# yyNoBug/VAE_segmentation

Hardware: AMD Instinct MI355X
Metric: 3D train-step volumes/sec at 96^3 batch=2 (joint VAE+seg) (higher is better)
Workload: dtype bf16; 1 GPU; configs[1]: 96^3 joint VAE+seg training step (joint_train), batch=2/GPU, bf16 activations + fp32 accumulate, SGD momentum 0.9, VAE frozen, HIP-graph replay; global_batch=2, parallelism=dp1, activation_recomputation=False, tail_in_graph=True, nranks=1, grad_exchange=none (1 rank)

## Files before the change

include/vaeseg.h:

```cpp
#ifndef VAESEG_H
#define VAESEG_H
#include <stddef.h>
#include <stdint.h>

#ifdef __cplusplus
extern "C" {
#endif

#define VS_VERSION 500

enum { VS_F32 = 0, VS_BF16 = 1, VS_F16 = 2, VS_F32X3 = 3  };
#ifndef VS_STAT_SLOTS
#define VS_STAT_SLOTS 4
#endif
enum { VS_OK = 0, VS_EINVAL = -1, VS_ESHAPE = -2, VS_EDTYPE = -3, VS_EWORKSPACE = -4, VS_EALIGN = -5 };

enum {
    VS_CONV_K3 = 0,
    VS_CONV_K2S2 = 1,
    VS_CONV_T2S2 = 2,
    VS_WGRAD_SLABS = 16,
    VS_CONV_UP = 3
};

// ... 85 lines not shown
    long long wgrad_f32_tiles;
    long long wgrad_group_wgs;
    long long wgrad_big_min_voxels;
} vs_config;
int vs_config_bytes(void);
int vs_config_from_env(vs_config* c);
int vs_get_config(vs_config* out);
int vs_set_config(const vs_config* cfg);
int vs_conv_k3_bwd_data_applied_supported(int n, int d, int h, int w, int c_in, int m_out, int dtype);
int vs_conv_k3_bwd_data_applied(const void* x, const void* w_packed, void* y, const void* mask_x, const double* mask_stats, double* sums,
                                unsigned int* sync, unsigned int* fault, int n, int d, int h, int w, int c_in, int m_out, int dtype, float eps, void* stream);
int vs_conv_s2_bwd_data_applied_supported(int n, int d, int h, int w, int c_in, int m_out, int scatter, int dtype);
int vs_conv_s2_bwd_data_applied(const void* x, const void* w_packed, void* y, const void* mask_x, const double* mask_stats, double* sums, const void* add,
                                unsigned int* sync, unsigned int* fault, int n, int d, int h, int w, int c_in, int m_out, int scatter, int dtype, float eps,
                                void* stream);
typedef struct vs_chain_layer {
    const void* x;
    const double* x_stats;
    const void* w_packed;
    void* y;
    double* y_stats;
    const void* mask_x;
    const double* mask_stats;
    double* sums;
    int c_in, m_out;
    int apply;
    int reserved_;
} vs_chain_layer;
int vs_conv_k3_chain_supported(int n, int d, int h, int w, int c_max, int dtype);
long long vs_conv_k3_chain_sync_bytes(int n);
// ... 35 lines not shown
int vs_bias_grad_acc(const void* g, float* db, long long rows, int c_ch, int c_real, int dtype, int accumulate, void* stream);

int vs_instnorm_stats(const void* x, double* stats, int n, long long voxels, int c, int dtype, void* stream);
int vs_instnorm_relu_fwd(const void* x, const double* x_stats, const void* x2, const double* x2_stats,
                         void* out, int n, long long voxels, int c, int dtype, float eps, void* stream);
int vs_instnorm_relu_bwd_reduce(const void* g, const void* x, const double* x_stats, double* sums,
                                int n, long long voxels, int c, int dtype, float eps, void* stream);
int vs_instnorm_relu_bwd_apply(const void* g, const void* x, const double* x_stats, const double* sums,
                               void* gx, int n, long long voxels, int c, int dtype, float eps, void* stream);
int vs_instnorm_relu_bwd_apply_add(const void* g, const void* x, const double* x_stats, const double* sums, const void* add,
                                   void* gx, int n, long long voxels, int c, int dtype, float eps, void* stream);
int vs_zero_fill(void* p, long long bytes, void* stream);
int vs_instnorm_relu_bwd_pair(const void* g, const void* x1, const double* x1_stats, double* sums1, void* gx1,
                              const void* x2, const double* x2_stats, double* sums2, void* gx2, int n, long long voxels,
                              int c, int dtype, float eps, void* stream);

enum { VS_NORM_INSTANCE = 0, VS_NORM_BATCH = 1, VS_NORM_BATCH_EVAL = 2, VS_NORM_NONE = 3 };
enum { VS_ACT_RELU = 0, VS_ACT_SOFTPLUS = 1 };
int vs_norm_tables(const double* stats, int n, int c, int c_real, double count, int mode, float eps, float momentum,
                   float* running_mean, float* running_var, long long* num_batches_tracked, float* mean, float* rstd, void* stream);
int vs_norm_act_fwd(const void* x, const float* mean, const float* rstd, const float* gamma, const float* beta, void* y, int n,
                    long long voxels, int c, int c_real, int act, int dtype, void* stream);
int vs_norm_act_bwd_reduce(const void* g, const void* x, const float* mean, const float* rstd, const float* gamma, const float* beta,
                           double* sums, int n, long long voxels, int c, int c_real, int act, int dtype, void* stream);
int vs_norm_act_bwd_finish(const double* sums, int n, int c, int c_real, double count, int mode, const float* rstd, const float* gamma,
                           float* coef, float* dgamma, float* dbeta, void* stream);
int vs_norm_act_bwd_apply(const void* g, const void* x, const float* mean, const float* rstd, const float* gamma, const float* beta,
                          const float* coef, void* dx, int n, long long voxels, int c, int c_real, int act, int dtype, void* stream);

int vs_gsnorm_fwd(const void* x, void* y, long long rows, int c, int num_group, int dtype, void* stream);
// ... 197 lines not shown
```

vae_segmentation_amd/csrc/conv_api.hip:

```cpp
#include <stdlib.h>
#include "igemm_dispatch.h"

int g1_dispatch_k3_f32(const G1Params& p, int ck, int mt, int epi, int tiles, int row_tiles, hipStream_t s);
int g1_dispatch_k3_bf16(const G1Params& p, int ck, int mt, int epi, int tiles, int row_tiles, hipStream_t s);
int g1_dispatch_k3_f16(const G1Params& p, int ck, int mt, int epi, int tiles, int row_tiles, hipStream_t s);
int g1_dispatch_k3_x3(const G1Params& p, int ck, int mt, int epi, int tiles, int row_tiles, hipStream_t s);
int g1_k3_fa_supported(const G1Params& p, int ck, int mt, int lazy_in);
int g1_k3_ea_supported(const G1Params& p, int ck, int mt, long long wgs);
int k3x_fa_supported(const G1Params& p, int ck, int mt);
int k3x_ea_supported(const G1Params& p, int ck, int mt, long long wgs);
int k3tw_slab_count(int n, int d, int h, int w);
int k2s2_scatter8_launch(const G1Params& p, int dtype, hipStream_t stream);

extern "C" int vs_conv_k3_f32_limbs(int d, int h, int w, int c_in) {
    const int on = vs_cfg().f32_limbs;
    if (!on) return 0;
    const int small = vs_cfg().k3_small;
    if (small && c_in % 32 == 0 && c_in <= 1024 && (long long)(d + 2) * (h + 2) * (w + 2) <= 512) return 0;
    return 1;
}

struct ConvTiles { int ck, mt, row_tiles; bool limbs; };

static ConvTiles k3_tiles(G1Params& p, int dtype, int ck, int mt, int rows16, long long tiles) {
// ... 30 lines not shown
static inline bool wide_layer(int c_in, int m_out) { return c_in > 256 || m_out > 256; }

static int shape_status(int n, int d, int h, int w_, int c_in, int dtype, bool misaligned = false) {
    if (n <= 0 || d <= 0 || h <= 0 || w_ <= 0) return VS_ESHAPE;
    if (!(c_in == 8 || c_in == 16 || (c_in % 32 == 0 && c_in > 0 && c_in <= VS_MAX_CHANNELS))) return VS_ESHAPE;
    if (!vs_dtype_ok(dtype)) return VS_EDTYPE;
    if (misaligned) return VS_EALIGN;
    return (double)n * d * h * w_ * c_in >= 2147483648.0 ? VS_ESHAPE : VS_OK;
}

static int check_common(const void* x, const void* w, int n, int d, int h, int w_, int c_in, int dtype) {
    if (!x || !w) return VS_EINVAL;
    return shape_status(n, d, h, w_, c_in, dtype, ((uintptr_t)x & 15) || ((uintptr_t)w & 15));
}

enum { X_STATS = 1, BIAS = 2, SUMS = 4, FA = 8, WGRAD = 16, EA = 32 };
struct ConvAsk { int n, d, h, w, c_in, m_out, kind, dtype, parts; };

struct ConvPlan {
    ConvAsk ask;
    G1Params g;
    ConvTiles t;
    long long tiles;
    int status;
    bool fa_ok, ea_ok, wg_ok;
    bool stream8;
};

static void g1_ea_plan(ConvPlan& pl, long long wgs) {
    pl.ea_ok = pl.t.mt == 16 && wgs <= 256;
    if (pl.ask.parts & EA) pl.g.ea_items = pl.g.tiles_per_sample * pl.t.row_tiles;
}

static ConvPlan plan_begin(const ConvAsk& a, int rows) {
    ConvPlan pl{};
    pl.ask = a;
    pl.status = shape_status(a.n, a.d, a.h, a.w, a.c_in, a.dtype);
    if (!pl.status && (a.m_out <= 0 || a.m_out % 8)) pl.status = VS_EINVAL;
    if (!pl.status && a.m_out > VS_MAX_CHANNELS) pl.status = VS_ESHAPE;
    if (pl.status) return pl;
    G1Params& p = pl.g;
    p.N = a.n; p.D = a.d; p.H = a.h; p.W = a.w;
    p.C = a.c_in; p.M = a.m_out;
    p.rb_total = (rows + 15) / 16;
    pl.t.ck = a.c_in < 32 ? a.c_in : 32;
    p.nch = a.c_in / pl.t.ck;
    p.inv_count_in = 1.0 / ((double)a.d * a.h * a.w);
    return pl;
}

static ConvPlan plan_gather(const ConvAsk& a) {
    ConvPlan pl = plan_begin(a, a.m_out);
    const bool k3 = a.kind == VS_CONV_K3, sums = a.parts & SUMS, fa = a.parts & FA, ea = a.parts & EA;
    if (!pl.status && !k3 && a.kind != VS_CONV_K2S2) pl.status = VS_EINVAL;
    if (!pl.status && wide_layer(a.c_in, a.m_out) && (a.parts & (EA | FA | WGRAD))) pl.status = VS_ESHAPE;
    if (!pl.status && !k3 && ((a.d | a.h | a.w) & 1)) pl.status = VS_ESHAPE;
    if (pl.status) return pl;
    G1Params& p = pl.g;
    const int ck = pl.t.ck;
    if (k3) {
        p.Do = a.d; p.Ho = a.h; p.Wo = a.w;
        p.tyn = (a.h + 3) / 4; p.txn = (a.w + 15) / 16;
        p.tiles_per_sample = ((a.d + 3) / 4) * p.tyn * p.txn;
    } else {
        p.Do = a.d / 2; p.Ho = a.h / 2; p.Wo = a.w / 2;
        p.tiles_per_sample = vs_ceil_div((long long)p.Do * p.Ho * p.Wo, 256);
        if (ck == 32 && p.nch >= 2 && (long long)p.tiles_per_sample * a.n * p.rb_total <= 64) {
            p.tiles_per_sample = vs_ceil_div((long long)p.Do * p.Ho * p.Wo, 64);
            p.tyn = 64;
        }
// ... 5 lines not shown
    if (k3 && fa && ck == 32 && mt == 16 && rows16 % 32 == 0) mt = 32;
    pl.t = k3 ? k3_tiles(p, a.dtype, ck, mt, rows16, pl.tiles) : ConvTiles{ck, mt, rows16 / mt, false};
    const long long wgs = pl.tiles * pl.t.row_tiles;
    if (!k3) {
        g1_ea_plan(pl, wgs);
    } else if (a.dtype != VS_F32) {
        pl.fa_ok = g1_k3_fa_supported(p, pl.t.ck, pl.t.mt, sums) != 0;
        pl.ea_ok = g1_k3_ea_supported(p, pl.t.ck, pl.t.mt, wgs) != 0;
        pl.wg_ok = vs_cfg().fuse_wgrad && a.c_in == 8 && a.m_out == 8 && a.n * 8 <= 192 && (double)a.n * a.d * a.h * a.w * 16 < 2147483648.0 &&
                   vs_k3_toeplitz(8, 8, 27, a.dtype);
    } else if (pl.t.limbs) {
        pl.fa_ok = k3x_fa_supported(p, pl.t.ck, pl.t.mt) != 0;
        pl.ea_ok = k3x_ea_supported(p, pl.t.ck, pl.t.mt, wgs) != 0;
    }
    pl.ea_ok = pl.ea_ok && sums && !fa && vs_cfg().epilogue_apply;
    if ((fa && !pl.fa_ok) || (ea && !pl.ea_ok) || ((a.parts & WGRAD) && !pl.wg_ok)) pl.status = VS_ESHAPE;
    return pl;
}

static ConvPlan plan_scatter(const ConvAsk& a) {
    ConvPlan pl = plan_begin(a, 8 * a.m_out);
    const bool sums = a.parts & SUMS, ea = a.parts & EA;
    if (!pl.status && wide_layer(a.c_in, a.m_out) && ea) pl.status = VS_ESHAPE;
    if (pl.status) return pl;
    G1Params& p = pl.g;
    p.Do = a.d; p.Ho = a.h; p.Wo = a.w;
    p.inv_count_out = 1.0 / (8.0 * a.d * a.h * a.w);
    p.tiles_per_sample = vs_ceil_div((long long)a.d * a.h * a.w, 256);
    pl.tiles = (long long)p.tiles_per_sample * a.n;
    pl.stream8 = !ea && vs_cfg().k2s2_stream && sums && a.c_in == 8 && a.m_out == 8 && a.dtype != VS_F32 && !(a.parts & (BIAS | X_STATS));
    const int rows16 = p.rb_total * 16;
// ... 140 lines not shown
    return plan_s2_applied(n, d, h, w, c_in, m_out, scatter, dtype).status == VS_OK;
}

extern "C" int vs_conv_s2_bwd_data_applied(const void* x, const void* w_packed, void* y, const void* mask_x, const double* mask_stats, double* sums, const void* add,
                                           unsigned int* sync, unsigned int* fault, int n, int d, int h, int w, int c_in, int m_out, int scatter, int dtype, float eps,
                                           void* stream) {
    if (!mask_x || !mask_stats || !sums || !sync || !fault) return VS_EINVAL;
    if (((uintptr_t)sync & 127) || ((uintptr_t)fault & 3) || (add && ((uintptr_t)add & 15))) return VS_EALIGN;
    const ConvPlan pl = plan_s2_applied(n, d, h, w, c_in, m_out, scatter, dtype);
    if (pl.status) return VS_ESHAPE;
    G1Params p = bwd_params(pl, x, w_packed, y, mask_x, mask_stats, sums, eps);
    p.ea_sync = sync; p.ea_fault = fault; p.ea_add = add;
    return launch_conv(pl, p, stream);
}

extern "C" int vs_conv_k3_softmax2_fwd(const void* x, const double* x_stats, const void* w_packed, const float* bias,
                                       float* prob, int n, int d, int h, int w, int c_in, int dtype, float eps,
                                       void* stream) {
    return vs_conv_k3_softmax2_dropout_fwd(x, x_stats, w_packed, bias, prob, n, d, h, w, c_in, dtype, eps, 0.f, 0ull, stream);
}

extern "C" int vs_conv_k3_softmax2_dropout_fwd(const void* x, const double* x_stats, const void* w_packed, const float* bias,
                                               float* prob, int n, int d, int h, int w, int c_in, int dtype, float eps,
                                               float drop_p, unsigned long long drop_seed, void* stream) {
    return vs_conv_k3_softmax2_cl_fwd(x, x_stats, w_packed, bias, prob, nullptr, n, d, h, w, c_in, dtype, eps, drop_p, drop_seed, stream);
}

extern "C" int vs_conv_k3_softmax2_cl_fwd(const void* x, const double* x_stats, const void* w_packed, const float* bias, float* prob, void* prob_cl,
                                          int n, int d, int h, int w, int c_in, int dtype, float eps, float drop_p, unsigned long long drop_seed, void* stream) {
    if (drop_p < 0.f || drop_p >= 1.f) return VS_EINVAL;
// ... 12 lines not shown
```

vae_segmentation_amd/csrc/igemm.h:

```cpp
#pragma once
#include <type_traits>
#include "common.h"
#include "handoff.h"

enum { G1_K3 = 0, G1_K2S2 = 1, G1_PW = 2 };
enum { EPI_RAW = 0, EPI_SOFTMAX2 = 1, EPI_SCATTER = 2 };

struct G1Params {
    const void* x;
    const double* x_stats;
    const void* wp;
    const float* bias;
    void* y;
    double* y_stats;
    float* prob;
    const void* mask_x;
    const double* mask_stats;
    double* sums;
    double inv_count_out;
    float drop_p;
    unsigned long long drop_seed;
    int N, D, H, W;
    int Do, Ho, Wo;
    int C;
    int M;
    int rb_total;
    int nch;
    int tiles_per_sample;
    int tyn, txn;
    float eps;
    double inv_count_in;
    unsigned int fd_m[3], fd_s[3];
    const void* fa_x;
    const double* fa_sums;
    void* fa_dx;
    const void* up_taps;
    const float* up_btab;
    int up_co;
    float* wg_ws;
    const float* sm_prob;
    const float* sm_gprob;
    const void* sm_gcl;
    double* wg_bias;
    unsigned int* ea_sync;
    unsigned int* ea_fault;
    int ea_items;
    const void* ea_add;
};

#define G1_LDS_MEAN 0
#define G1_LDS_RSTD 2048
#define G1_LDS_RED 4096
#define G1_LDS_BYTES 6144
#define G1_TILE_VOX 648

template <typename T, int CK>
__device__ __forceinline__ u32x4 act_transform(u32x4 raw, const float* s_mean, const float* s_rstd, int c0) {
    constexpr int EPL = ET<T>::EPL;
    float v[EPL];
    frag_unpack(raw, v, (T*)nullptr);
#pragma unroll
    for (int j = 0; j < EPL; ++j) {
        float t = (v[j] - s_mean[c0 + j]) * s_rstd[c0 + j];
        v[j] = t > 0.f ? t : 0.f;
    }
    return frag_pack(v, (T*)nullptr);
}

template <typename T, int CK, int KIND, int MT, int EPI, bool LIMB = false, bool EA = false>
__global__ __launch_bounds__(256) void g1_kernel(const G1Params p) {
    using E = ET<T>;
    constexpr int EPL = E::EPL, KG = E::KG;
    static_assert(!LIMB || sizeof(T) == 4, "limb arithmetic: fp32 storage");
    static_assert(KIND == G1_K2S2 || KIND == G1_PW, "the 3x3x3 kernels live in igemm_k3b.h / igemm_k3.h");
    static_assert(EPI == EPI_RAW || EPI == EPI_SCATTER, "softmax epilogue: 3x3x3 kernels only");
    constexpr int NTAPS = KIND == G1_K2S2 ? 8 : 1;
    constexpr int NKG = (NTAPS * CK + KG - 1) / KG;
    constexpr int RB = MT / 16;
    constexpr int CKB = CK * (int)sizeof(T);
    constexpr int TPK = KG > CK ? KG / CK : 1;
    constexpr int KPT = KG > CK ? 1 : CK / KG;
    extern __shared__ __attribute__((aligned(16))) char smem[];
    float* s_mean = (float*)(smem + G1_LDS_MEAN);
    float* s_rstd = (float*)(smem + G1_LDS_RSTD);
    float* s_red = (float*)(smem + G1_LDS_RED);

    const int tid = threadIdx.x;
    const int lane = tid & 63;
    const int wave = tid >> 6;
    const int col = lane & 15;
    const int g = lane >> 4;
    const int n = blockIdx.x / p.tiles_per_sample;
    const int tile = blockIdx.x - n * p.tiles_per_sample;
    const int rb0 = blockIdx.y * RB;
    const bool has_stats = p.x_stats != nullptr;
    const T* __restrict__ xin = (const T*)p.x;

    if (has_stats) {
        for (int c = tid; c < p.C; c += 256) {
            float m, r;
            stats_to_mean_rstd(p.x_stats, (size_t)n * p.C + c, (size_t)p.N * p.C, p.inv_count_in, p.eps, m, r);
            s_mean[c] = m;
            s_rstd[c] = r;
        }
    }
    if (p.sums != nullptr) {
        for (int c = tid; c < p.M; c += 256) {
            float m, r;
            stats_to_mean_rstd(p.mask_stats, (size_t)n * p.M + c, (size_t)p.N * p.M, p.inv_count_out, p.eps, m, r);
            s_mean[c] = m;
            s_rstd[c] = r;
        }
    }
    const bool splitw = KIND == G1_K2S2 && CK == 32 && p.tyn == 64;
    const int cwave = splitw ? 0 : wave;
    const int ctile = splitw ? 64 : 256;
    long long gofs[4];
    bool cvalid[4];
    int oz[4], oy[4], ox[4];
    {
        const int vcol = p.Do * p.Ho * p.Wo;
#pragma unroll
        for (int cg = 0; cg < 4; ++cg) {
            int v = tile * ctile + cwave * 64 + cg * 16 + col;
            cvalid[cg] = v < vcol;
            if (!cvalid[cg]) v = 0;
// ... 247 lines not shown

    auto out_elem = [&](int rb, int cg, int& m_out, bool& valid) -> size_t {
        const int row = (rb0 + rb) * 16 + 4 * g;
        int m = row, tap = 0;
        if constexpr (EPI == EPI_SCATTER) { tap = row / p.M; m = row - tap * p.M; }
        const bool rvalid = EPI == EPI_SCATTER ? (tap < 8) : (row < p.M);
        m_out = m;
        valid = rvalid && cvalid[cg];
        if constexpr (EPI == EPI_SCATTER) {
            const int dz = (tap >> 2) & 1, dy = (tap >> 1) & 1, dx = tap & 1;
            return ((((size_t)n * (2 * p.D) + 2 * oz[cg] + dz) * (2 * p.H) + 2 * oy[cg] + dy) * (2 * p.W) + 2 * ox[cg] + dx) * p.M + m;
        } else {
            return ((((size_t)n * p.Do + oz[cg]) * p.Ho + oy[cg]) * p.Wo + ox[cg]) * p.M + m;
        }
    };
    constexpr int MKW = sizeof(T) == 4 ? 4 : 2;
    unsigned int mkv[RB][4][MKW];
    constexpr bool ea = EA;
    static_assert(!EA || MT == 16, "epilogue apply: 16-row workgroups");
    unsigned int adv[EA ? RB : 1][4][MKW];
    if (p.sums != nullptr) {
#pragma unroll
        for (int rb = 0; rb < RB; ++rb)
#pragma unroll
            for (int cg = 0; cg < 4; ++cg) {
                int m; bool ok;
                const size_t e = out_elem(rb, cg, m, ok);
#pragma unroll
                for (int i = 0; i < MKW; ++i) { mkv[rb][cg][i] = 0u; if constexpr (EA) adv[rb][cg][i] = 0u; }
                if (ok) {
// ... 132 lines not shown
                float xv[4], av[4], o[4];
                widen4<T>(mkv[rb][cg], xv);
                widen4<T>(adv[rb][cg], av);
#pragma unroll
                for (int r = 0; r < 4; ++r) {
                    const float gv = E::rnd(acc[rb][cg][r] + bvq[rb][r]);
                    o[r] = vs_in_bwd_apply1(gv, xv[r], tb[r][0], tb[r][1], tb[r][2], tb[r][3]);
                    if (p.ea_add != nullptr) o[r] = E::rnd(o[r]) + av[r];
                }
                store4<T>(yout + e, o);
            }
        }
    }
}

template <typename T, int CK, int KIND, int MT, int EPI, bool LIMB = false, bool EA = false>
static int g1_launch(const G1Params& p, int tiles_total, int row_tiles, hipStream_t stream) {
    constexpr size_t lds = G1_LDS_BYTES + (KIND == G1_K2S2 && CK == 32 ? (size_t)3 * (MT / 16) * 4 * 64 * 16 : 0);
    auto kern = g1_kernel<T, CK, KIND, MT, EPI, LIMB, EA>;
    hipLaunchKernelGGL(kern, dim3(tiles_total, row_tiles), dim3(256), lds, stream, p);
    VS_CHECK_LAUNCH();
    return VS_OK;
}
```

vae_segmentation_amd/csrc/igemm_dispatch.h:

```cpp
#pragma once
#include "igemm.h"

int g1_dispatch_k2s2(const G1Params& p, int dtype, int ck, int mt, int tiles, int row_tiles, hipStream_t s);
int g1_dispatch_pw(const G1Params& p, int dtype, int ck, int mt, int tiles, int row_tiles, hipStream_t s);

#define G1_CASE(T, CKV, KIND, MTV, EPI) \
    if (ck == CKV && mt == MTV) return g1_launch<T, CKV, KIND, MTV, EPI>(p, tiles, row_tiles, s);

#define G1_ALL_MT(T, CKV, KIND, EPI) \
    G1_CASE(T, CKV, KIND, 16, EPI) G1_CASE(T, CKV, KIND, 32, EPI) G1_CASE(T, CKV, KIND, 64, EPI)

#define G1_ALL(T, KIND, EPI) G1_ALL_MT(T, 8, KIND, EPI) G1_ALL_MT(T, 16, KIND, EPI) G1_ALL_MT(T, 32, KIND, EPI)
#define G1L_CASE(CKV, KIND, MTV, EPI) \
    if (ck == CKV && mt == MTV) return g1_launch<float, CKV, KIND, MTV, EPI, true>(p, tiles, row_tiles, s);
#define G1L_ALL_MT(CKV, KIND, EPI) G1L_CASE(CKV, KIND, 16, EPI) G1L_CASE(CKV, KIND, 32, EPI) G1L_CASE(CKV, KIND, 64, EPI)
#define G1L_ALL(KIND, EPI) G1L_ALL_MT(8, KIND, EPI) G1L_ALL_MT(16, KIND, EPI) G1L_ALL_MT(32, KIND, EPI)
#define G1E_ALL(T, KIND, EPI, LIMBV) \
    if (p.ea_sync != nullptr) { \
        if (mt == 16 && ck == 8) return g1_launch<T, 8, KIND, 16, EPI, LIMBV, true>(p, tiles, row_tiles, s); \
        if (mt == 16 && ck == 16) return g1_launch<T, 16, KIND, 16, EPI, LIMBV, true>(p, tiles, row_tiles, s); \
        if (mt == 16 && ck == 32) return g1_launch<T, 32, KIND, 16, EPI, LIMBV, true>(p, tiles, row_tiles, s); \
        return VS_ESHAPE; \
    }
static inline bool g1_f32_limbs() {
    const int on = vs_cfg().f32_limbs;
    const int g1 = vs_cfg().g1_limbs;
    return on != 0 && g1 != 0;
}
```

vae_segmentation_amd/csrc/igemm_g1_f16.hip:

```cpp
#include "igemm_dispatch.h"
int g1_dispatch_k2s2_f16(const G1Params& p, int ck, int mt, int tiles, int row_tiles, hipStream_t s) {
    G1E_ALL(vs_half, G1_K2S2, EPI_RAW, false)
    G1_ALL(vs_half, G1_K2S2, EPI_RAW)
    return VS_ESHAPE;
}
int g1_dispatch_pw_f16(const G1Params& p, int ck, int mt, int tiles, int row_tiles, hipStream_t s) {
    G1E_ALL(vs_half, G1_PW, EPI_SCATTER, false)
    G1_ALL(vs_half, G1_PW, EPI_SCATTER)
    return VS_ESHAPE;
}
```

vae_segmentation_amd/csrc/igemm_k2s2.hip:

```cpp
#include <stdlib.h>
#include "igemm_dispatch.h"
int g1_dispatch_k2s2_f16(const G1Params& p, int ck, int mt, int tiles, int row_tiles, hipStream_t s);
int g1_dispatch_k2s2(const G1Params& p, int dtype, int ck, int mt, int tiles, int row_tiles, hipStream_t s) {
    if (dtype == VS_F32) { if (g1_f32_limbs()) { G1E_ALL(float, G1_K2S2, EPI_RAW, true) G1L_ALL(G1_K2S2, EPI_RAW) } else { G1E_ALL(float, G1_K2S2, EPI_RAW, false) G1_ALL(float, G1_K2S2, EPI_RAW) } }
    else if (dtype == VS_BF16) { G1E_ALL(unsigned short, G1_K2S2, EPI_RAW, false) G1_ALL(unsigned short, G1_K2S2, EPI_RAW) }
    else if (dtype == VS_F16) return g1_dispatch_k2s2_f16(p, ck, mt, tiles, row_tiles, s);
    return VS_ESHAPE;
}
```

vae_segmentation_amd/csrc/norm.hip:

```cpp
#include "common.h"

#define NB_MAX_C 512

template <typename T>
struct RowIter {
    int fx, fy, frags, rows_per_it;
    __device__ RowIter(int c) {
        frags = c / ET<T>::EPL;
        fx = threadIdx.x % frags;
        fy = threadIdx.x / frags;
        rows_per_it = 256 / frags;
    }
    __device__ bool active() const { return fy < rows_per_it; }
};

__device__ __forceinline__ void load_mean_rstd(const double* stats, int n, int c, double inv_count, float eps,
                                               float* s_mean, float* s_rstd) {
    const size_t pairs = (size_t)gridDim.y * c;
    for (int i = threadIdx.x; i < c; i += blockDim.x) {
        float m = 0.f, r = 1.f;
        if (stats) stats_to_mean_rstd(stats, (size_t)n * c + i, pairs, inv_count, eps, m, r);
        s_mean[i] = m;
        s_rstd[i] = r;
    }
// ... 340 lines not shown
extern "C" int vs_instnorm_relu_bwd_pair(const void* g, const void* x1, const double* x1_stats, double* sums1, void* gx1,
                                         const void* x2, const double* x2_stats, double* sums2, void* gx2, int n, long long voxels,
                                         int c, int dtype, float eps, void* stream) {
    int rc = check_cl(x1, n, voxels, c, dtype);
    if (rc) return rc;
    if (!g || !x2 || !x1_stats || !x2_stats || !sums1 || !sums2 || !gx1 || !gx2) return VS_EINVAL;
    InBwdPair a;
    a.x[0] = x1; a.x[1] = x2; a.xs[0] = x1_stats; a.xs[1] = x2_stats; a.sums[0] = sums1; a.sums[1] = sums2; a.gx[0] = gx1; a.gx[1] = gx2;
    const double inv = 1.0 / (double)voxels;
    dim3 grid(row_blocks(voxels, c, dtype), n, 2);
    dispatch_t(dtype, [&](auto* tag) {
        using T = TAG_T(tag);
        hipLaunchKernelGGL(in_relu_bwd_reduce2_kernel<T>, grid, dim3(256), red_lds(dtype, 2), (hipStream_t)stream, (const T*)g, a, voxels, c, inv, eps);
    });
    VS_CHECK_LAUNCH();
    const int rpi = 256 / (c / (dtype == VS_F32 ? 4 : 8));
    long long gb = (voxels + (long long)rpi * 4 - 1) / ((long long)rpi * 4);
    const long long gcap = 2048 / (2 * n) > 0 ? 2048 / (2 * n) : 1;
    if (gb > gcap) gb = gcap;
    dim3 grid2((unsigned)gb, n, 2);
    dispatch_t(dtype, [&](auto* tag) {
        using T = TAG_T(tag);
        hipLaunchKernelGGL(in_relu_bwd_apply2_kernel<T>, grid2, dim3(256), 0, (hipStream_t)stream, (const T*)g, a, voxels, c, inv, eps);
    });
    VS_CHECK_LAUNCH();
    return VS_OK;
}

extern "C" int vs_bias_grad(const void* g, float* db, long long rows, int c_ch, int c_real, int dtype, void* stream) {
    return vs_bias_grad_acc(g, db, rows, c_ch, c_real, dtype, 0, stream);
// ... 286 lines not shown
```

vae_segmentation_amd/modules.py:

```python
import torch
import torch.nn as nn

from . import ops

_DEFAULT_DTYPE = torch.float32


def set_default_kernel_dtype(dtype):
    global _DEFAULT_DTYPE
    if dtype not in ops.KERNEL_DTYPES:
        raise TypeError("kernel dtype must be torch.float32, torch.bfloat16 or torch.float16")
    _DEFAULT_DTYPE = dtype


def set_kernel_dtype(module, dtype):
    if dtype not in ops.KERNEL_DTYPES:
        raise TypeError("kernel dtype must be torch.float32, torch.bfloat16 or torch.float16")
    for m in module.modules():
        if hasattr(m, "kernel_dtype"):
            m.kernel_dtype = dtype
    return module


class Act:
# ... 106 lines not shown
        a = _conv_norm_act(self.conv, 0, a)
        return _as_tensor(a, self.out_ch) if wrapped else a


class Up(nn.Module):

    def __init__(self, in_ch, out_ch, norm_type=2, kernal_size=(2, 2, 2), stride=(2, 2, 2), soft=False):
        super().__init__()
        if tuple(kernal_size) != (2, 2, 2) or tuple(stride) != (2, 2, 2):
            raise NotImplementedError("native transposed conv is written for kernel 2, stride 2")
        self.conv = nn.Sequential(nn.ConvTranspose3d(in_ch, in_ch, kernal_size, stride=stride, padding=0),
                                  DoubleConv(in_ch, out_ch, norm_type, soft=False))
        self.out_ch = out_ch
        self.kernel_dtype = _DEFAULT_DTYPE

    def forward(self, x):
        a, wrapped = _as_act(x, self.kernel_dtype)
        t, dc = self.conv[0], self.conv[1]
        if dc.lazy_head() and ops.up_composed_ok(a.raw, t, dc.conv[0]):
            y, ys = ops.UpConvK3.apply(a.raw, a.stats, t.weight, t.bias, dc.conv[0].weight, dc.conv[0].bias)
            a = dc(Act(y, ys), _start=3)
        else:
            a = dc(Act(ops.ConvT2S2.apply(a.raw, a.stats, t.weight, t.bias), None))
        return _as_tensor(a, self.out_ch) if wrapped else a


class Down(nn.Module):

    def __init__(self, in_ch, out_ch, norm_type=2, kernal_size=(2, 2, 2), stride=(2, 2, 2), soft=False):
        super().__init__()
        if tuple(kernal_size) != (2, 2, 2) or tuple(stride) != (2, 2, 2):
            raise NotImplementedError("native strided conv is written for kernel 2, stride 2")
        self.conv = nn.Sequential(nn.Conv3d(in_ch, in_ch, kernal_size, stride=stride, padding=0),
# ... 16 lines not shown
    enabled = bool(enabled)
    if enabled == _RECOMPUTE[0]:
        return
    _RECOMPUTE[0] = enabled
    if enabled:
        _RECOMPUTE_SAVED_GROUPING[0] = bool(ops._GROUP["enabled"])
        ops.set_wgrad_grouping(False)
    else:
        ops.set_wgrad_grouping(_RECOMPUTE_SAVED_GROUPING[0])


def _has_training_batchnorm(blk):
    return any(isinstance(m, nn.BatchNorm3d) and m.training for m in blk.modules())


def _run_block(blk, a):
    if not (_RECOMPUTE[0] and torch.is_grad_enabled() and a.raw.requires_grad):
        return blk(a)
    if _has_training_batchnorm(blk):
        return blk(a)
    from torch.utils.checkpoint import checkpoint

    def run(raw, stats):
        out = blk(Act(raw, stats))
        return out.raw, out.stats

    marks = getattr(a.raw, "_vs_defer_apply", False)

    def run_marked(raw, stats):
        if marks:
            raw._vs_defer_apply = True
        return run(raw, stats)

    raw, stats = checkpoint(run_marked, a.raw, a.stats, use_reentrant=False, preserve_rng_state=False)
    return Act(raw, stats)


def _check_n_class(n_class):
    if not 1 <= int(n_class) <= 8:
        raise NotImplementedError("native softmax / label kernels hold n_class in one 8-channel fragment: 1..8, got %r" % (n_class,))


def _dropout(a, p):
    if not p:
        return a
    x = ops.Materialize.apply(a.raw, a.stats, None, None) if a.stats is not None else a.raw
    return Act(ops.Dropout.apply(x, float(p), ops.next_dropout_seed()), None)


# ... 91 lines not shown

    def forward(self, data_dict, in_key, out_key, dropout=0.0):
        x = data_dict[in_key]
        ops._require_cuda(x)
        if any(s % 16 for s in x.shape[2:]):
            raise ValueError("Segmentation needs spatial sizes that are multiples of 16, got %s" % (tuple(x.shape[2:]),))
        ops.stats_arena_begin(x.device)
        a = Act(ops.PackPlanar.apply(x, self.kernel_dtype), None)
        x1 = self.in_block(a)
        x2 = _run_block(self.down1, x1)
        x3 = _run_block(self.down2, x2)
        x4 = _run_block(self.down3, x3)
        x5 = _run_block(self.down4, x4)
        u = _dropout(_run_block(self.up2, x5), dropout)
        u = _run_block(self.up3, u)
        u = _dropout(Act(ops.Materialize.apply(u.raw, u.stats, x3.raw, x3.stats, True), None), dropout)
        u = _run_block(self.up4, u)
        u = _dropout(Act(ops.Materialize.apply(u.raw, u.stats, x2.raw, x2.stats, True), None), dropout)
        u = _dropout(_run_block(self.up5, u), dropout)
        if u.stats is not None:
            ops.mark_defer_apply(u.raw, self.up5.conv[1].conv[6])
        if dropout:
            data_dict[out_key] = ops.out_block_softmax(u.raw, u.stats, self.out_block.weight, self.out_block.bias,
                                                       float(dropout), ops.next_dropout_seed())
        else:
            data_dict[out_key] = ops.out_block_softmax(u.raw, u.stats, self.out_block.weight, self.out_block.bias)
        return data_dict


class Joint(nn.Module):

    def __init__(self, models, vae_forward_scale=0.0, vae_decoder_dropout=0.0, seg_dropout=0.0):
        super().__init__()
        self.Seg = models[0]
# ... 144 lines not shown
```

vae_segmentation_amd/ops.py:

```python
import ctypes as _ctypes
import os
import weakref as _weakref

import torch

from . import _lib
from ._lib import (VS_BF16, VS_CONV_K2S2, VS_CONV_K3, VS_CONV_UP, VS_F16, VS_F32, VS_PACK_ROWS_D0, VS_PACK_ROWS_D1_FLIP,
                   VS_PACK_SCATTER_D1, _contig, _p, _require_cuda, _stream, check, lib)
from .volume import *
from .volume import (PATCH_CHUNK, PATCH_LABEL_DTYPES, PATCH_MAX_CLASSES, PATCH_MAX_SOURCES, patch_gather, patch_index,
                     patch_pick)

_DT_TORCH = {VS_F32: torch.float32, VS_BF16: torch.bfloat16, VS_F16: torch.float16}
_DT_VS = {v: k for k, v in _DT_TORCH.items()}
KERNEL_DTYPES = tuple(_DT_VS)
VS_F32X3 = 3
F32X3 = "f32x3"
_DT_TORCH[VS_F32X3] = F32X3
_DT_VS[F32X3] = VS_F32X3
_F32_LIMBS = bool(lib.vs_conv_k3_f32_limbs(96, 96, 96, 8))


def k3_pack_dtype(x):
    if x.dtype == torch.float32 and lib.vs_conv_k3_f32_limbs(x.shape[1], x.shape[2], x.shape[3], x.shape[4]):
# ... 1296 lines not shown
        gx = gw = gb = None
        if ctx.needs_input_grad[0]:
            wpb = pack_weight_cached(weight, VS_PACK_ROWS_D0, gy.shape[-1], gy.dtype)
            if xs is not None:
                gx = conv_bwd_data_lazy(gy, wpb, x, xs, VS_CONV_K2S2, defer=ctx.defer)
            else:
                gx, _ = conv_gather(gy, None, wpb, None, x.shape[-1], VS_CONV_K2S2, False)
        if ctx.needs_input_grad[2]:
            gw, gb = _side_grads(weight, (gy, x, xs), (x, xs, gy, None, cin, cout, VS_CONV_K2S2),
                                 (gy, cout) if ctx.has_bias and ctx.needs_input_grad[3] else None, ctx.bias_ref)
        elif ctx.has_bias and ctx.needs_input_grad[3]:
            gb = bias_grad(gy, cout)
        return gx, None, gw, gb


FUSE_UP = os.environ.get("VS_FUSE_UP", "1") != "0"
FUSE_UP_MIN_VOXELS = int(os.environ.get("VS_FUSE_UP_MIN_VOXELS", "1000"))
_FUT = os.environ.get("VS_FUSE_UP_TRAINABLE", "")
FUSE_UP_TRAINABLE = _FUT != "0"
FUSE_UP_TRAINABLE_MIN_VOXELS = 0 if _FUT == "1" else int(os.environ.get("VS_FUSE_UP_TRAINABLE_MIN_VOXELS", "500000"))


def _up_stamp(wt, bt, w3):
    return (wt._version, wt.data_ptr(), w3._version, w3.data_ptr(), None if bt is None else (bt._version, bt.data_ptr()),
            _TRAIN_EPOCH[0] if (w3.requires_grad or wt.requires_grad) else _PACK_EPOCH[0])


_UP_TRAINABLE = {}


# ... 858 lines not shown
```

Before: 891.8 volumes/s.

## Fuse skip-add instnorm-relu into transposed-conv and its backward with paired stats

Adds a SkipConvT2S2 autograd op for the up4/up5 decoder blocks. Its forward applies the two-input instnorm+relu and feeds the result straight into the stride-2 transposed conv. Its backward uses a new g1 kernel variant that computes the data gradient while reducing instnorm-relu backward sums for both skip inputs at once, followed by a paired apply kernel. The goal is to drop the separate Materialize pass and the standalone reduction passes over the data gradient, at the cost of extra LDS and register pressure in the pair epilogue and some new dispatch complexity.

```diff
diff --git a/include/vaeseg.h b/include/vaeseg.h
--- a/include/vaeseg.h
+++ b/include/vaeseg.h
@@ -123,6 +123,9 @@
 int vs_conv_s2_bwd_data_applied(const void* x, const void* w_packed, void* y, const void* mask_x, const double* mask_stats, double* sums, const void* add,
                                 unsigned int* sync, unsigned int* fault, int n, int d, int h, int w, int c_in, int m_out, int scatter, int dtype, float eps,
                                 void* stream);
+int vs_conv_s2_bwd_data_pair_supported(int n, int d, int h, int w, int c_in, int m_out, int dtype);
+int vs_conv_s2_bwd_data_pair(const void* x, const void* w_packed, void* y, const void* mask_x, const double* mask_stats, double* sums, const void* mask2_x,
+                             const double* mask2_stats, double* sums2, int n, int d, int h, int w, int c_in, int m_out, int dtype, float eps, void* stream);
 typedef struct vs_chain_layer {
     const void* x;
     const double* x_stats;
@@ -188,6 +191,9 @@
 int vs_instnorm_relu_bwd_pair(const void* g, const void* x1, const double* x1_stats, double* sums1, void* gx1,
                               const void* x2, const double* x2_stats, double* sums2, void* gx2, int n, long long voxels,
                               int c, int dtype, float eps, void* stream);
+int vs_instnorm_relu_bwd_pair_apply(const void* g, const void* x1, const double* x1_stats, const double* sums1, void* gx1,
+                                    const void* x2, const double* x2_stats, const double* sums2, void* gx2, int n, long long voxels,
+                                    int c, int dtype, float eps, void* stream);
 
 enum { VS_NORM_INSTANCE = 0, VS_NORM_BATCH = 1, VS_NORM_BATCH_EVAL = 2, VS_NORM_NONE = 3 };
 enum { VS_ACT_RELU = 0, VS_ACT_SOFTPLUS = 1 };
diff --git a/vae_segmentation_amd/csrc/conv_api.hip b/vae_segmentation_amd/csrc/conv_api.hip
--- a/vae_segmentation_amd/csrc/conv_api.hip
+++ b/vae_segmentation_amd/csrc/conv_api.hip
@@ -68,7 +68,7 @@
     return shape_status(n, d, h, w_, c_in, dtype, ((uintptr_t)x & 15) || ((uintptr_t)w & 15));
 }
 
-enum { X_STATS = 1, BIAS = 2, SUMS = 4, FA = 8, WGRAD = 16, EA = 32 };
+enum { X_STATS = 1, BIAS = 2, SUMS = 4, FA = 8, WGRAD = 16, EA = 32, PAIR = 64 };
 struct ConvAsk { int n, d, h, w, c_in, m_out, kind, dtype, parts; };
 
 struct ConvPlan {
@@ -78,6 +78,7 @@
     long long tiles;
     int status;
     bool fa_ok, ea_ok, wg_ok;
+    bool pair_ok;
     bool stream8;
 };
 
@@ -105,9 +106,9 @@
 
 static ConvPlan plan_gather(const ConvAsk& a) {
     ConvPlan pl = plan_begin(a, a.m_out);
-    const bool k3 = a.kind == VS_CONV_K3, sums = a.parts & SUMS, fa = a.parts & FA, ea = a.parts & EA;
+    const bool k3 = a.kind == VS_CONV_K3, sums = a.parts & SUMS, fa = a.parts & FA, ea = a.parts & EA, pair = a.parts & PAIR;
     if (!pl.status && !k3 && a.kind != VS_CONV_K2S2) pl.status = VS_EINVAL;
-    if (!pl.status && wide_layer(a.c_in, a.m_out) && (a.parts & (EA | FA | WGRAD))) pl.status = VS_ESHAPE;
+    if (!pl.status && wide_layer(a.c_in, a.m_out) && (a.parts & (EA | FA | WGRAD | PAIR))) pl.status = VS_ESHAPE;
     if (!pl.status && !k3 && ((a.d | a.h | a.w) & 1)) pl.status = VS_ESHAPE;
     if (pl.status) return pl;
     G1Params& p = pl.g;
@@ -143,7 +144,8 @@
         pl.ea_ok = k3x_ea_supported(p, pl.t.ck, pl.t.mt, wgs) != 0;
     }
     pl.ea_ok = pl.ea_ok && sums && !fa && vs_cfg().epilogue_apply;
-    if ((fa && !pl.fa_ok) || (ea && !pl.ea_ok) || ((a.parts & WGRAD) && !pl.wg_ok)) pl.status = VS_ESHAPE;
+    pl.pair_ok = !k3 && sums && !ea && !fa && a.dtype != VS_F32 && pl.t.mt == 16;
+    if ((fa && !pl.fa_ok) || (ea && !pl.ea_ok) || ((a.parts & WGRAD) && !pl.wg_ok) || (pair && !pl.pair_ok)) pl.status = VS_ESHAPE;
     return pl;
 }
 
@@ -314,6 +316,24 @@
     return launch_conv(pl, p, stream);
 }
 
+static ConvPlan plan_s2_pair(int n, int d, int h, int w, int c_in, int m_out, int dtype) {
+    return plan_gather({n, d, h, w, c_in, m_out, VS_CONV_K2S2, dtype, SUMS | PAIR});
+}
+extern "C" int vs_conv_s2_bwd_data_pair_supported(int n, int d, int h, int w, int c_in, int m_out, int dtype) {
+    return plan_s2_pair(n, d, h, w, c_in, m_out, dtype).status == VS_OK;
+}
+
+extern "C" int vs_conv_s2_bwd_data_pair(const void* x, const void* w_packed, void* y, const void* mask_x, const double* mask_stats, double* sums, const void* mask2_x,
+                                        const double* mask2_stats, double* sums2, int n, int d, int h, int w, int c_in, int m_out, int dtype, float eps, void* stream) {
+    if (!mask_x || !mask_stats || !sums || !mask2_x || !mask2_stats || !sums2 || sums == sums2) return VS_EINVAL;
+    if (((uintptr_t)mask_x & 15) || ((uintptr_t)mask2_x & 15)) return VS_EALIGN;
+    const ConvPlan pl = plan_s2_pair(n, d, h, w, c_in, m_out, dtype);
+    if (pl.status) return pl.status == VS_EDTYPE || pl.status == VS_EINVAL ? pl.status : VS_ESHAPE;
+    G1Params p = bwd_params(pl, x, w_packed, y, mask_x, mask_stats, sums, eps);
+    p.mask2_x = mask2_x; p.mask2_stats = mask2_stats; p.sums2 = sums2;
+    return launch_conv(pl, p, stream);
+}
+
 extern "C" int vs_conv_k3_softmax2_fwd(const void* x, const double* x_stats, const void* w_packed, const float* bias,
                                        float* prob, int n, int d, int h, int w, int c_in, int dtype, float eps,
                                        void* stream) {
diff --git a/vae_segmentation_amd/csrc/igemm.h b/vae_segmentation_amd/csrc/igemm.h
--- a/vae_segmentation_amd/csrc/igemm.h
+++ b/vae_segmentation_amd/csrc/igemm.h
@@ -31,9 +31,9 @@
     float eps;
     double inv_count_in;
     unsigned int fd_m[3], fd_s[3];
-    const void* fa_x;
-    const double* fa_sums;
-    void* fa_dx;
+    union { const void* fa_x; const void* mask2_x; };
+    union { const double* fa_sums; const double* mask2_stats; };
+    union { void* fa_dx; double* sums2; };
     const void* up_taps;
     const float* up_btab;
     int up_co;
@@ -52,6 +52,7 @@
 #define G1_LDS_RSTD 2048
 #define G1_LDS_RED 4096
 #define G1_LDS_BYTES 6144
+#define G1_LDS_T2_BYTES 4096
 #define G1_TILE_VOX 648
 
 template <typename T, int CK>
@@ -67,10 +68,23 @@
     return frag_pack(v, (T*)nullptr);
 }
 
-template <typename T, int CK, int KIND, int MT, int EPI, bool LIMB = false, bool EA = false>
+template <int CK, int KIND, int MT>
+constexpr size_t g1_t2_offset() { return G1_LDS_BYTES + (KIND == G1_K2S2 && CK == 32 ? (size_t)3 * (MT / 16) * 4 * 64 * 16 : 0); }
+
+__device__ __forceinline__ double row16_sum_d(double v) {
+#define VS_DPP_D(ctrl) { const long long b = __builtin_bit_cast(long long, v); \
+        const int lo = __builtin_amdgcn_update_dpp(0, (int)b, ctrl, 0xF, 0xF, true), hi = __builtin_amdgcn_update_dpp(0, (int)(b >> 32), ctrl, 0xF, 0xF, true); \
+        v += __builtin_bit_cast(double, ((long long)hi << 32) | (long long)(unsigned int)lo); }
+    VS_DPP_D(0xB1) VS_DPP_D(0x4E) VS_DPP_D(0x141) VS_DPP_D(0x140)
+#undef VS_DPP_D
+    return v;
+}
+
+template <typename T, int CK, int KIND, int MT, int EPI, bool LIMB = false, bool EA = false, bool PAIR = false>
 __global__ __launch_bounds__(256) void g1_kernel(const G1Params p) {
     using E = ET<T>;
     constexpr int EPL = E::EPL, KG = E::KG;
+    static_assert(!PAIR || (KIND == G1_K2S2 && EPI == EPI_RAW && MT == 16 && !EA && !LIMB && sizeof(T) == 2), "pair sums: the stride-2 gather, 16-row workgroups, 16-bit storage");
     static_assert(!LIMB || sizeof(T) == 4, "limb arithmetic: fp32 storage");
     static_assert(KIND == G1_K2S2 || KIND == G1_PW, "the 3x3x3 kernels live in igemm_k3b.h / igemm_k3.h");
     static_assert(EPI == EPI_RAW || EPI == EPI_SCATTER, "softmax epilogue: 3x3x3 kernels only");
@@ -84,6 +98,8 @@
     float* s_mean = (float*)(smem + G1_LDS_MEAN);
     float* s_rstd = (float*)(smem + G1_LDS_RSTD);
     float* s_red = (float*)(smem + G1_LDS_RED);
+    float* s_mean2 = (float*)(smem + g1_t2_offset<CK, KIND, MT>());
+    float* s_rstd2 = s_mean2 + 512;
 
     const int tid = threadIdx.x;
     const int lane = tid & 63;
@@ -110,6 +126,14 @@
             stats_to_mean_rstd(p.mask_stats, (size_t)n * p.M + c, (size_t)p.N * p.M, p.inv_count_out, p.eps, m, r);
             s_mean[c] = m;
             s_rstd[c] = r;
+        }
+    }
+    if constexpr (PAIR) {
+        for (int c = tid; c < p.M; c += 256) {
+            float m, r;
+            stats_to_mean_rstd(p.mask2_stats, (size_t)n * p.M + c, (size_t)p.N * p.M, p.inv_count_out, p.eps, m, r);
+            s_mean2[c] = m;
+            s_rstd2[c] = r;
         }
     }
     const bool splitw = KIND == G1_K2S2 && CK == 32 && p.tyn == 64;
@@ -387,6 +411,76 @@
             return ((((size_t)n * p.Do + oz[cg]) * p.Ho + oy[cg]) * p.Wo + ox[cg]) * p.M + m;
         }
     };
+    if constexpr (PAIR) {
+        unsigned int mk1[4][2], mk2[4][2];
+        size_t eo[4];
+        bool eok[4];
+#pragma unroll
+        for (int cg = 0; cg < 4; ++cg) {
+            int m;
+            eo[cg] = out_elem(0, cg, m, eok[cg]);
+            mk1[cg][0] = mk1[cg][1] = mk2[cg][0] = mk2[cg][1] = 0u;
+            if (eok[cg]) {
+                const u32x2 xa = *(const u32x2*)((const T*)p.mask_x + eo[cg]);
+                const u32x2 xb = *(const u32x2*)((const T*)p.mask2_x + eo[cg]);
+                mk1[cg][0] = xa[0]; mk1[cg][1] = xa[1];
+                mk2[cg][0] = xb[0]; mk2[cg][1] = xb[1];
+            }
+        }
+        const int row = rb0 * 16 + 4 * g;
+        const bool rvalid = row < p.M;
+        float bv[4], pm[2][4], pr[2][4];
+        double sa[2][4], sb[2][4];
+#pragma unroll
+        for (int r = 0; r < 4; ++r) {
+            bv[r] = (p.bias && rvalid) ? p.bias[row + r] : 0.f;
+            pm[0][r] = rvalid ? s_mean[row + r] : 0.f;  pr[0][r] = rvalid ? s_rstd[row + r] : 1.f;
+            pm[1][r] = rvalid ? s_mean2[row + r] : 0.f; pr[1][r] = rvalid ? s_rstd2[row + r] : 1.f;
+            sa[0][r] = sa[1][r] = sb[0][r] = sb[1][r] = 0.0;
+        }
+#pragma unroll
+        for (int cg = 0; cg < 4; ++cg) {
+            if (!eok[cg]) continue;
+            float v[4], xv[2][4];
+#pragma unroll
+            for (int r = 0; r < 4; ++r) v[r] = E::rnd(acc[0][cg][r] + bv[r]);
+            store4<T>(yout + eo[cg], v);
+            widen4<T>(mk1[cg], xv[0]);
+            widen4<T>(mk2[cg], xv[1]);
+#pragma unroll
+            for (int k = 0; k < 2; ++k)
+#pragma unroll
+                for (int r = 0; r < 4; ++r) {
+                    const float xh = (xv[k][r] - pm[k][r]) * pr[k][r];
+                    const float gm = xh > 0.f ? v[r] : 0.f;
+                    sa[k][r] += (double)gm;
+                    sb[k][r] += (double)gm * (double)xh;
+                }
+        }
+        double* s_redd = (double*)s_red;
+#pragma unroll
+        for (int k = 0; k < 2; ++k)
+#pragma unroll
+            for (int r = 0; r < 4; ++r) {
+                const double a = row16_sum_d(sa[k][r]), b = row16_sum_d(sb[k][r]);
+                if (col == 0) {
+                    s_redd[((wave * 16 + 4 * g + r) * 2 + k) * 2 + 0] = a;
+                    s_redd[((wave * 16 + 4 * g + r) * 2 + k) * 2 + 1] = b;
+                }
+            }
+        __syncthreads();
+        if (tid < 64) {
+            const int k = tid >> 5, lr = (tid >> 1) & 15, st = tid & 1;
+            const int orow = rb0 * 16 + lr;
+            if (orow < p.M) {
+                double tot = 0.0;
+#pragma unroll
+                for (int w = 0; w < 4; ++w) tot += s_redd[((w * 16 + lr) * 2 + k) * 2 + st];
+                stat_add(k ? p.sums2 : p.sums, (size_t)n * p.M + orow, (size_t)p.N * p.M, st, tot);
+            }
+        }
+        return;
+    }
     constexpr int MKW = sizeof(T) == 4 ? 4 : 2;
     unsigned int mkv[RB][4][MKW];
     constexpr bool ea = EA;
@@ -549,10 +643,10 @@
     }
 }
 
-template <typename T, int CK, int KIND, int MT, int EPI, bool LIMB = false, bool EA = false>
+template <typename T, int CK, int KIND, int MT, int EPI, bool LIMB = false, bool EA = false, bool PAIR = false>
 static int g1_launch(const G1Params& p, int tiles_total, int row_tiles, hipStream_t stream) {
-    constexpr size_t lds = G1_LDS_BYTES + (KIND == G1_K2S2 && CK == 32 ? (size_t)3 * (MT / 16) * 4 * 64 * 16 : 0);
-    auto kern = g1_kernel<T, CK, KIND, MT, EPI, LIMB, EA>;
+    constexpr size_t lds = g1_t2_offset<CK, KIND, MT>() + (PAIR ? G1_LDS_T2_BYTES : 0);
+    auto kern = g1_kernel<T, CK, KIND, MT, EPI, LIMB, EA, PAIR>;
     hipLaunchKernelGGL(kern, dim3(tiles_total, row_tiles), dim3(256), lds, stream, p);
     VS_CHECK_LAUNCH();
     return VS_OK;
diff --git a/vae_segmentation_amd/csrc/igemm_dispatch.h b/vae_segmentation_amd/csrc/igemm_dispatch.h
--- a/vae_segmentation_amd/csrc/igemm_dispatch.h
+++ b/vae_segmentation_amd/csrc/igemm_dispatch.h
@@ -22,6 +22,13 @@
         if (mt == 16 && ck == 32) return g1_launch<T, 32, KIND, 16, EPI, LIMBV, true>(p, tiles, row_tiles, s); \
         return VS_ESHAPE; \
     }
+#define G1P_ALL(T) \
+    if (p.sums2 != nullptr) { \
+        if (mt == 16 && ck == 8) return g1_launch<T, 8, G1_K2S2, 16, EPI_RAW, false, false, true>(p, tiles, row_tiles, s); \
+        if (mt == 16 && ck == 16) return g1_launch<T, 16, G1_K2S2, 16, EPI_RAW, false, false, true>(p, tiles, row_tiles, s); \
+        if (mt == 16 && ck == 32) return g1_launch<T, 32, G1_K2S2, 16, EPI_RAW, false, false, true>(p, tiles, row_tiles, s); \
+        return VS_ESHAPE; \
+    }
 static inline bool g1_f32_limbs() {
     const int on = vs_cfg().f32_limbs;
     const int g1 = vs_cfg().g1_limbs;
diff --git a/vae_segmentation_amd/csrc/igemm_g1_f16.hip b/vae_segmentation_amd/csrc/igemm_g1_f16.hip
--- a/vae_segmentation_amd/csrc/igemm_g1_f16.hip
+++ b/vae_segmentation_amd/csrc/igemm_g1_f16.hip
@@ -1,5 +1,6 @@
 #include "igemm_dispatch.h"
 int g1_dispatch_k2s2_f16(const G1Params& p, int ck, int mt, int tiles, int row_tiles, hipStream_t s) {
+    G1P_ALL(vs_half)
     G1E_ALL(vs_half, G1_K2S2, EPI_RAW, false)
     G1_ALL(vs_half, G1_K2S2, EPI_RAW)
     return VS_ESHAPE;
diff --git a/vae_segmentation_amd/csrc/igemm_k2s2.hip b/vae_segmentation_amd/csrc/igemm_k2s2.hip
--- a/vae_segmentation_amd/csrc/igemm_k2s2.hip
+++ b/vae_segmentation_amd/csrc/igemm_k2s2.hip
@@ -2,8 +2,9 @@
 #include "igemm_dispatch.h"
 int g1_dispatch_k2s2_f16(const G1Params& p, int ck, int mt, int tiles, int row_tiles, hipStream_t s);
 int g1_dispatch_k2s2(const G1Params& p, int dtype, int ck, int mt, int tiles, int row_tiles, hipStream_t s) {
+    if (p.sums2 != nullptr && dtype == VS_F32) return VS_EDTYPE;
     if (dtype == VS_F32) { if (g1_f32_limbs()) { G1E_ALL(float, G1_K2S2, EPI_RAW, true) G1L_ALL(G1_K2S2, EPI_RAW) } else { G1E_ALL(float, G1_K2S2, EPI_RAW, false) G1_ALL(float, G1_K2S2, EPI_RAW) } }
-    else if (dtype == VS_BF16) { G1E_ALL(unsigned short, G1_K2S2, EPI_RAW, false) G1_ALL(unsigned short, G1_K2S2, EPI_RAW) }
+    else if (dtype == VS_BF16) { G1P_ALL(unsigned short) G1E_ALL(unsigned short, G1_K2S2, EPI_RAW, false) G1_ALL(unsigned short, G1_K2S2, EPI_RAW) }
     else if (dtype == VS_F16) return g1_dispatch_k2s2_f16(p, ck, mt, tiles, row_tiles, s);
     return VS_ESHAPE;
 }
diff --git a/vae_segmentation_amd/csrc/norm.hip b/vae_segmentation_amd/csrc/norm.hip
--- a/vae_segmentation_amd/csrc/norm.hip
+++ b/vae_segmentation_amd/csrc/norm.hip
@@ -378,6 +378,18 @@
         hipLaunchKernelGGL(in_relu_bwd_reduce2_kernel<T>, grid, dim3(256), red_lds(dtype, 2), (hipStream_t)stream, (const T*)g, a, voxels, c, inv, eps);
     });
     VS_CHECK_LAUNCH();
+    return vs_instnorm_relu_bwd_pair_apply(g, x1, x1_stats, sums1, gx1, x2, x2_stats, sums2, gx2, n, voxels, c, dtype, eps, stream);
+}
+
+extern "C" int vs_instnorm_relu_bwd_pair_apply(const void* g, const void* x1, const double* x1_stats, const double* sums1, void* gx1,
+                                               const void* x2, const double* x2_stats, const double* sums2, void* gx2, int n, long long voxels,
+                                               int c, int dtype, float eps, void* stream) {
+    int rc = check_cl(x1, n, voxels, c, dtype);
+    if (rc) return rc;
+    if (!g || !x2 || !x1_stats || !x2_stats || !sums1 || !sums2 || !gx1 || !gx2) return VS_EINVAL;
+    InBwdPair a;
+    a.x[0] = x1; a.x[1] = x2; a.xs[0] = x1_stats; a.xs[1] = x2_stats; a.sums[0] = (double*)sums1; a.sums[1] = (double*)sums2; a.gx[0] = gx1; a.gx[1] = gx2;
+    const double inv = 1.0 / (double)voxels;
     const int rpi = 256 / (c / (dtype == VS_F32 ? 4 : 8));
     long long gb = (voxels + (long long)rpi * 4 - 1) / ((long long)rpi * 4);
     const long long gcap = 2048 / (2 * n) > 0 ? 2048 / (2 * n) : 1;
diff --git a/vae_segmentation_amd/modules.py b/vae_segmentation_amd/modules.py
--- a/vae_segmentation_amd/modules.py
+++ b/vae_segmentation_amd/modules.py
@@ -144,9 +144,21 @@
         self.out_ch = out_ch
         self.kernel_dtype = _DEFAULT_DTYPE
 
-    def forward(self, x):
+    def skip_ok(self, a, skip):
+        t, dc = self.conv[0], self.conv[1]
+        if not (isinstance(a, Act) and isinstance(skip, Act)) or (dc.lazy_head() and ops.up_composed_ok(a.raw, t, dc.conv[0])):
+            return False
+        return ops.skip_convt_ok(a.raw, a.stats, skip.raw, skip.stats, t.weight)
+
+    def forward(self, x, skip=None):
         a, wrapped = _as_act(x, self.kernel_dtype)
         t, dc = self.conv[0], self.conv[1]
+        if skip is not None:
+            if self.skip_ok(a, skip):
+                y, _ = ops.SkipConvT2S2.apply(a.raw, a.stats, skip.raw, skip.stats, t.weight, t.bias, True)
+                a = dc(Act(y, None))
+                return _as_tensor(a, self.out_ch) if wrapped else a
+            a = Act(ops.Materialize.apply(a.raw, a.stats, skip.raw, skip.stats, True), None)
         if dc.lazy_head() and ops.up_composed_ok(a.raw, t, dc.conv[0]):
             y, ys = ops.UpConvK3.apply(a.raw, a.stats, t.weight, t.bias, dc.conv[0].weight, dc.conv[0].bias)
             a = dc(Act(y, ys), _start=3)
@@ -193,25 +205,27 @@
     return any(isinstance(m, nn.BatchNorm3d) and m.training for m in blk.modules())
 
 
-def _run_block(blk, a):
+def _run_block(blk, a, skip=None):
+    extra = () if skip is None else (skip,)
     if not (_RECOMPUTE[0] and torch.is_grad_enabled() and a.raw.requires_grad):
-        return blk(a)
+        return blk(a, *extra)
     if _has_training_batchnorm(blk):
-        return blk(a)
+        return blk(a, *extra)
     from torch.utils.checkpoint import checkpoint
 
-    def run(raw, stats):
-        out = blk(Act(raw, stats))
+    def run(raw, stats, *sk):
+        out = blk(Act(raw, stats), *([Act(sk[0], sk[1])] if sk else []))
         return out.raw, out.stats
 
     marks = getattr(a.raw, "_vs_defer_apply", False)
 
-    def run_marked(raw, stats):
+    def run_marked(raw, stats, *sk):
         if marks:
             raw._vs_defer_apply = True
-        return run(raw, stats)
-
-    raw, stats = checkpoint(run_marked, a.raw, a.stats, use_reentrant=False, preserve_rng_state=False)
+        return run(raw, stats, *sk)
+
+    sk = () if skip is None else (skip.raw, skip.stats)
+    raw, stats = checkpoint(run_marked, a.raw, a.stats, *sk, use_reentrant=False, preserve_rng_state=False)
     return Act(raw, stats)
 
 
@@ -333,10 +347,17 @@
         x5 = _run_block(self.down4, x4)
         u = _dropout(_run_block(self.up2, x5), dropout)
         u = _run_block(self.up3, u)
-        u = _dropout(Act(ops.Materialize.apply(u.raw, u.stats, x3.raw, x3.stats, True), None), dropout)
-        u = _run_block(self.up4, u)
-        u = _dropout(Act(ops.Materialize.apply(u.raw, u.stats, x2.raw, x2.stats, True), None), dropout)
-        u = _dropout(_run_block(self.up5, u), dropout)
+        if not dropout and self.up4.skip_ok(u, x3):
+            u = _run_block(self.up4, u, x3)
+        else:
+            u = _dropout(Act(ops.Materialize.apply(u.raw, u.stats, x3.raw, x3.stats, True), None), dropout)
+            u = _run_block(self.up4, u)
+        if not dropout and self.up5.skip_ok(u, x2):
+            u = _run_block(self.up5, u, x2)
+        else:
+            u = _dropout(Act(ops.Materialize.apply(u.raw, u.stats, x2.raw, x2.stats, True), None), dropout)
+            u = _run_block(self.up5, u)
+        u = _dropout(u, dropout)
         if u.stats is not None:
             ops.mark_defer_apply(u.raw, self.up5.conv[1].conv[6])
         if dropout:
diff --git a/vae_segmentation_amd/ops.py b/vae_segmentation_amd/ops.py
--- a/vae_segmentation_amd/ops.py
+++ b/vae_segmentation_amd/ops.py
@@ -1334,6 +1334,81 @@
         return gx, None, gw, gb
 
 
+FUSE_SKIP = os.environ.get("VS_FUSE_SKIP", "1") != "0"
+
+
+def skip_convt_ok(x, xs, x2, x2s, weight):
+    if not FUSE_SKIP or xs is None or x2 is None or x2s is None or x.dtype == torch.float32 or x.shape != x2.shape or x.dtype != x2.dtype:
+        return False
+    n, d, h, w, c = x.shape
+    try:
+        return bool(lib.vs_conv_s2_bwd_data_pair_supported(n, 2 * d, 2 * h, 2 * w, cpad(weight.shape[1]), c, vs_dtype(x)))
+    except AttributeError:
+        return False
+
+
+class SkipConvT2S2(torch.autograd.Function):
+
+    @staticmethod
+    def forward(ctx, x, xs, x2, x2s, weight, bias, park_second=False):
+        _require_cuda(x, weight)
+        n, c = x.shape[0], x.shape[-1]
+        a = torch.empty_like(x)
+        with _timed("in_relu_fwd_kernel<%s>" % _tname(x), 3 * x.numel() * _esize(x), 6.0 * x.numel(), str(tuple(x.shape))):
+            check(lib.vs_instnorm_relu_fwd(x.data_ptr(), xs.data_ptr(), x2.data_ptr(), x2s.data_ptr(), a.data_ptr(), n, x.numel() // (n * c), c, vs_dtype(x),
+                                           EPS_IN, _stream()), "instnorm_relu_fwd")
+        wp = pack_weight_cached(weight, VS_PACK_SCATTER_D1, c, x.dtype)
+        y = conv_scatter(a, None, wp, bias, cpad(weight.shape[1]))
+        ctx.save_for_backward(x, xs, x2, x2s, a, weight)
+        ctx.has_bias = bias is not None
+        ctx.bias_ref = bias
+        ctx.park_second = bool(park_second)
+        ctx.mark_non_differentiable(a)
+        ctx.set_materialize_grads(False)
+        return y, a
+
+    @staticmethod
+    def backward(ctx, gy, _ga):
+        x, xs, x2, x2s, a, weight = ctx.saved_tensors
+        gy = _contig(gy)
+        cin, cout = weight.shape[0], weight.shape[1]
+        g1 = g2 = gw = gb = None
+        if ctx.needs_input_grad[0] and ctx.needs_input_grad[2]:
+            wpb = pack_weight_cached(weight, VS_PACK_ROWS_D0, gy.shape[-1], gy.dtype)
+            gn, gd, gh, gw_, gc = gy.shape
+            n, c = x.shape[0], x.shape[-1]
+            dt = vs_dtype(x)
+            g = torch.empty_like(x)
+            s1, s2 = _new_stats(n, c, x.device), _new_stats(n, c, x.device)
+            kid = nb = fl = None
+            if PROFILE is not None:
+                kid = "g1_kernel<%s,%d,1,16,0>+pair" % (_tname(x), min(gc, 32))
+                nb = (gy.numel() + 3 * g.numel()) * _esize(x) + 8 * gc * c * _esize(x)
+                fl = 2.0 * (g.numel() // c) * 8 * gc * c
+            with _timed(kid, nb, fl, "bwd+pair gy%s->m%d" % (tuple(gy.shape), c)):
+                check(lib.vs_conv_s2_bwd_data_pair(gy.data_ptr(), wpb.data_ptr(), g.data_ptr(), x.data_ptr(), xs.data_ptr(), s1.data_ptr(), x2.data_ptr(),
+                                                   x2s.data_ptr(), s2.data_ptr(), gn, gd, gh, gw_, gc, c, dt, EPS_IN, _stream()), "conv_s2_bwd_data_pair")
+            g1, g2 = torch.empty_like(g), torch.empty_like(g)
+            with _timed("in_relu_bwd_apply2_kernel<%s>" % _tname(x), 5 * x.numel() * _esize(x), 12.0 * x.numel(), str(tuple(x.shape))):
+                check(lib.vs_instnorm_relu_bwd_pair_apply(g.data_ptr(), x.data_ptr(), xs.data_ptr(), s1.data_ptr(), g1.data_ptr(), x2.data_ptr(), x2s.data_ptr(),
+                                                          s2.data_ptr(), g2.data_ptr(), n, x.numel() // (n * c), c, dt, EPS_IN, _stream()),
+                      "instnorm_relu_bwd_pair_apply")
+        elif ctx.needs_input_grad[0] or ctx.needs_input_grad[2]:
+            wpb = pack_weight_cached(weight, VS_PACK_ROWS_D0, gy.shape[-1], gy.dtype)
+            g, _ = conv_gather(gy, None, wpb, None, x.shape[-1], VS_CONV_K2S2, False)
+            g1 = in_relu_bwd(g, x, xs, inplace=False) if ctx.needs_input_grad[0] else None
+            g2 = in_relu_bwd(g, x2, x2s, inplace=False) if ctx.needs_input_grad[2] else None
+        if g2 is not None and ctx.park_second and not torch.is_grad_enabled():
+            _park_gradient(x2, g2)
+            g2 = None
+        if ctx.needs_input_grad[4]:
+            gw, gb = _side_grads(weight, (gy, a, None), (a, None, gy, None, cin, cout, VS_CONV_K2S2),
+                                 (gy, cout) if ctx.has_bias and ctx.needs_input_grad[5] else None, ctx.bias_ref)
+        elif ctx.has_bias and ctx.needs_input_grad[5]:
+            gb = bias_grad(gy, cout)
+        return g1, None, g2, None, gw, gb, None
+
+
 FUSE_UP = os.environ.get("VS_FUSE_UP", "1") != "0"
 FUSE_UP_MIN_VOXELS = int(os.environ.get("VS_FUSE_UP_MIN_VOXELS", "1000"))
 _FUT = os.environ.get("VS_FUSE_UP_TRAINABLE", "")
```

Result: no change. 894.8 volumes/s, median of 6 (+0.3%).
